# babbu3682/MTD-GAN

Hardware: NVIDIA B200
Metric: train patches/s (64x64, bs20/GPU) (higher is better)
Workload: dtype f32

## Files before the change

include/mtdgan_b200.h:

```cpp
#ifndef MTDGAN_B200_H_
#define MTDGAN_B200_H_

#ifdef __cplusplus
extern "C" {
#endif

#define MTD_ACT_NONE_C 0
#define MTD_ACT_RELU_C 1
#define MTD_ACT_LEAKY_C 2

int mtd_abi_version(void);
int mtd_device_ok(void);
long long mtd_kernel_launch_count(void);
int mtd_set_pdl(int enabled);

int mtd_conv_pack_fwd(const float* w_ref, int transposed, int Cout, int Cin, int kh, int kw, float* out, void* stream);
int mtd_conv_pack_dgrad(const float* w_ref, int transposed, int Cout, int Cin, int kh, int kw, int stride, float* out,
                        void* stream);
int mtd_conv_pack_fwd_blocked(const float* w_ref, int transposed, int Cout, int Cin, int kh, int kw, int tf32, float* out,
                              void* stream);
int mtd_conv_pack_dgrad_blocked(const float* w_ref, int transposed, int Cout, int Cin, int kh, int kw, int stride, int tf32,
                                float* out, void* stream);
int mtd_conv_pack_batch_begin(void);
int mtd_conv_pack_batch_end(void* stream);
int mtd_conv_fwd(const float* x1, const float* x2, const float* wp, const float* bias, const float* scale, int scale_group,
                 float* y,
                 float* aux, const float* add1, const float* add2, int B, int H, int W, int C1, int C2, int N, int kh,
                 int kw, int stride, int pad, int pre_act, int post_act, float slope, void* stream);
int mtd_conv_dgrad(const float* dz, const float* wpd, float* dx, const float* scale, int scale_group, const float* add1,
                   const float* add2, const float* mask_src, int mask_act, float slope, int B, int H, int W, int Cin,
                   int Cout, int kh, int kw, int stride, int pad, void* stream);
int mtd_conv_wgrad(const float* x1, const float* x2, const float* dz, float* gp, int B, int H, int W, int C1, int C2,
                   int N, int kh, int kw, int stride, int pad, void* stream);
int mtd_conv_wgrad_finish(const float* gp, float* dw_ref, int transposed, int Cout, int Cin, int kh, int kw,
                          const float* w_ref, const float* u, const float* v, const float* inv_sigma, void* scratch,
                          void* stream);
int mtd_act_bwd_sn(const float* dy, const float* y, float* dz, float* dbias, const float* bias, double* zw,
                   const float* dz_scale, int groups, long long M, int N, int act, float slope, void* stream);
int mtd_wgrad_finish_chunk_elems(int taps, int cin);
int mtd_wgrad_finish_batched(const void* seg_tab, int n_segs, const void* dot_chunks, int n_dot_chunks, const void* head_chunks,
                             int n_head_chunks, double* dots, void* stream);
int mtd_act_bwd(const float* dy, const float* y, float* dz, float* dbias, int dbias_zeroed, long long M, int N, int act, float slope,
                void* stream);

int mtd_conv_fwd_tc_supported(int B, int H, int W, int C1, int C2, int N, int kh, int kw, int stride, int pad);
int mtd_tc_set_version(int version);
int mtd_tc_set_tuning(int bn, int sk_per);
int mtd_tc_set_c32(int enabled);
int mtd_tc_set_halo(int enabled);
int mtd_round_tf32(float* p, long long n, void* stream);
int mtd_conv_fwd_tc(const float* x1, const float* x2, const float* wp, const float* bias, const float* scale, int scale_group,
                    float* y,
                    float* aux, const float* add1, const float* add2, int B, int H, int W, int C1, int C2, int N, int kh,
                    int kw, int stride, int pad, int pre_act, int post_act, float slope, int passes, float* ws, long long ws_floats,
                    void* stream);
int mtd_conv_dgrad_tc(const float* dz, const float* wpd, float* dx, const float* scale, int scale_group, const float* add1,
                      const float* add2,
                      const float* mask_src, int mask_act, float slope, int B, int H, int W, int Cin, int Cout, int kh, int kw,
                      int stride, int pad, int passes, int cin_total, float* dx2, int c_split, float* ws, long long ws_floats,
                      void* stream);
int mtd_conv_wgrad_tc_supported(int B, int H, int W, int C1, int C2, int N, int kh, int kw, int stride, int pad);
int mtd_conv_wgrad_tc(const float* x1, const float* x2, const float* dz, float* gp, int B, int H, int W, int C1, int C2, int N,
                      int kh, int kw, int stride, int pad, int passes, void* stream);
int mtd_split_tf32(float* hi, float* lo, long long n, void* stream);

int mtd_fft_supported(int H, int W, int C);
long long mtd_fft_spec_elems(int B, int H, int W, int C);
long long mtd_fft_bwd_part_elems(int B, int W);
int mtd_fft_rows_fwd(const float* x, float* spec, int B, int H, int W, int C, void* stream);
int mtd_fft_cols_mix(const float* spec_in, float* spec_out, const float* w, const float* bias, int B, int H, int W,
                     int C, void* stream);
int mtd_fft_rows_inv(const float* spec, const float* add1, const float* add2, float* out, int B, int H, int W, int C,
                     void* stream);
int mtd_fft_cols_mix_bwd(const float* spec_x, const float* spec_g, float* spec_out, const float* w, const float* bias,
                         float* part, float* dw, float* db, int B, int H, int W, int C, void* stream);

int mtd_sn_rows_per_wtu_item(void);
int mtd_sn_power_iter(const void* layer_tab, int n_layers, const void* work_wtu, int n_wtu, const void* work_wv,
                      int n_wv, float* t_ws, long long t_elems, float* s_ws, float* u_snap, float* v_snap,
                      float* inv_sigma, int update, float eps, void* stream);

int mtd_upsample2x_fwd(const float* in, float* out, int B, int H, int W, int C, void* stream);
int mtd_upsample2x_bwd(const float* dout, float* din, int B, int H, int W, int C, void* stream);
int mtd_pixel_shuffle2(const float* in, float* out, int B, int H, int W, int C, int backward, void* stream);
int mtd_layout_transpose(const float* in, float* out, int B, int C, int HW, int to_nhwc, void* stream);
int mtd_clip01_fwd(const float* x, float* y, long long n, void* stream);
int mtd_clip01_bwd(const float* x, const float* dy, float* dx, long long n, void* stream);
int mtd_mul(const float* a, const float* b, float* out, long long n, void* stream);
int mtd_add3(const float* a, const float* b, const float* c, float* out, long long n, void* stream);

int mtd_nds_mask(const float* x, const float* y, unsigned char* mask, long long n, void* stream);
// ... 32 lines not shown
```

mtd-gan_b200/csrc/conv_simt.cu:

```cuda
#include <algorithm>
#include <string.h>
#include <vector>
#include "common.cuh"
#include "mtdgan_b200.h"

namespace {

constexpr int kMaxTaps = 16;

struct ConvArgs {
  const float* src1;
  const float* src2;
  int C1, C2;
  int B, H, W;
  const float* wp;
  int N, T;
  int Ho, Wo;
  int sy, sx;
  int dy[kMaxTaps], dx[kMaxTaps];
  float* out;
  int outH, outW, omy, omx, ooy, oox;
  const float* scale;
  long long scale_span;
  const float* bias;
// ... 1018 lines not shown
#pragma unroll
        for (int j = 0; j < TC; ++j) acc[i][j] = fmaf(av[i], bv[j], acc[i][j]);
    }
    if (has_next) store_tiles(buf ^ 1);
    __syncthreads();
    buf ^= 1;
  }
#pragma unroll
  for (int i = 0; i < TN; ++i) {
    int n = n0 + ty * TN + i;
    if (n >= a.N) continue;
#pragma unroll
    for (int j = 0; j < TC; ++j) {
      int c = c0 + tx * TC + j;
      if (c >= Ctot) continue;
      float* dst = a.gp + ((size_t)n * a.T + t) * Ctot + c;
      if (a.splits > 1) atomicAdd(dst, acc[i][j]);
      else *dst = acc[i][j];
    }
  }
}

int launch_wgrad(WgradArgs& a, cudaStream_t st) {
  const int Ctot = a.C1 + a.C2;
  const int M = a.B * a.Ho * a.Wo;
  if (M <= 0 || a.N <= 0 || Ctot <= 0 || a.T <= 0 || a.T > kMaxTaps) return MTD_EINVAL;
  bool vec = (a.C1 % 4 == 0) && (a.C2 % 4 == 0) && (a.N % 4 == 0) && mtd_aligned16(a.src1) &&
             mtd_aligned16(a.dz) && (a.C2 == 0 || mtd_aligned16(a.src2));
  bool thin_n = a.N <= 16, thin_c = Ctot <= 16;
  int BN = thin_n ? 16 : 64, BC = thin_c ? 16 : 64;
  dim3 grid((a.N + BN - 1) / BN, (Ctot + BC - 1) / BC, a.T);
  int tiles = grid.x * grid.y * grid.z;
  int target = 4 * mtd_sm_count();
  int splits = 1;
  if (tiles < target) splits = std::min((target + tiles - 1) / tiles, std::max(1, M / 64));
  if (splits > 256) splits = 256;
  a.splits = splits;
  grid.z = a.T * splits;
  if (splits > 1) MTD_CUDA(cudaMemsetAsync(a.gp, 0, (size_t)a.N * a.T * Ctot * sizeof(float), st));
#define WG_LAUNCH(TN_, TC_)                                                              \
  do {                                                                                   \
    if (vec) mtd_launch(conv_wgrad_kernel<TN_, TC_, true>, grid, 256, 0, st, a);                 \
    else mtd_launch(conv_wgrad_kernel<TN_, TC_, false>, grid, 256, 0, st, a);                    \
  } while (0)
  if (thin_n && thin_c) WG_LAUNCH(1, 1);
  else if (thin_n) WG_LAUNCH(1, 4);
  else if (thin_c) WG_LAUNCH(4, 1);
  else WG_LAUNCH(4, 4);
#undef WG_LAUNCH
  MTD_CHECK_LAUNCH();
  return MTD_OK;
}

__global__ void act_bwd_kernel(const float* __restrict__ dy, const float* __restrict__ y, float* __restrict__ dz,
                               float* __restrict__ dbias, size_t total, int N, int act, float slope) {
  mtd_pdl_prologue();
  extern __shared__ float colsum[];
  if (dbias) {
    for (int i = threadIdx.x; i < N; i += blockDim.x) colsum[i] = 0.f;
    __syncthreads();
  }
  size_t i = (size_t)blockIdx.x * blockDim.x + threadIdx.x;
  size_t stride = (size_t)gridDim.x * blockDim.x;
  const bool fixed = dbias && (stride % (size_t)N == 0);
  float priv = 0.f;
  for (; i < total; i += stride) {
    float g = dy[i];
    if (act != MTD_ACT_NONE) g *= mtd_act_grad(__ldg(y + i), act, slope);
    if (dz) dz[i] = g;
    if (dbias) {
      if (fixed) priv += g;
      else atomicAdd(&colsum[i % N], g);
    }
  }
  if (dbias) {
    if (fixed) {
      size_t first = (size_t)blockIdx.x * blockDim.x + threadIdx.x;
      atomicAdd(&colsum[first % N], priv);
    }
    __syncthreads();
    for (int c = threadIdx.x; c < N; c += blockDim.x) {
      float v = colsum[c];
      if (v != 0.f) atomicAdd(dbias + c, v);
    }
  }
}

__global__ void __launch_bounds__(256) act_bwd_v4_kernel(const float4* __restrict__ dy, const float4* __restrict__ y,
                                                         float4* __restrict__ dz, float* __restrict__ dbias, size_t total4,
                                                         int N4, int act, float slope) {
  mtd_pdl_prologue();
  extern __shared__ float colsum[];
  if (dbias) {
    for (int i = threadIdx.x; i < 4 * N4; i += blockDim.x) colsum[i] = 0.f;
    __syncthreads();
  }
  size_t i = (size_t)blockIdx.x * blockDim.x + threadIdx.x;
  const size_t stride = (size_t)gridDim.x * blockDim.x;
  const bool fixed = dbias && (stride % (size_t)N4 == 0);
  float4 priv = make_float4(0.f, 0.f, 0.f, 0.f);
  const size_t first = i;
  for (; i < total4; i += stride) {
    float4 g = __ldcs(dy + i);
    if (act != MTD_ACT_NONE) {
      const float4 t = __ldcs(y + i);
      g.x *= mtd_act_grad(t.x, act, slope); g.y *= mtd_act_grad(t.y, act, slope);
      g.z *= mtd_act_grad(t.z, act, slope); g.w *= mtd_act_grad(t.w, act, slope);
    }
    if (dz) dz[i] = g;
    if (dbias) {
      if (fixed) { priv.x += g.x; priv.y += g.y; priv.z += g.z; priv.w += g.w; }
      else {
        float* cs = colsum + 4 * (i % N4);
        atomicAdd(cs, g.x); atomicAdd(cs + 1, g.y); atomicAdd(cs + 2, g.z); atomicAdd(cs + 3, g.w);
      }
    }
  }
  if (dbias) {
    if (fixed && first < total4) {
      float* cs = colsum + 4 * (first % N4);
      atomicAdd(cs, priv.x); atomicAdd(cs + 1, priv.y); atomicAdd(cs + 2, priv.z); atomicAdd(cs + 3, priv.w);
    }
    __syncthreads();
    for (int c = threadIdx.x; c < 4 * N4; c += blockDim.x) {
      float v = colsum[c];
      if (v != 0.f) atomicAdd(dbias + c, v);
    }
  }
}

__global__ void __launch_bounds__(256) act_bwd_sn_kernel(const float4* __restrict__ dy, const float4* __restrict__ y,
                                                         float4* __restrict__ dz, float* __restrict__ dbias,
                                                         const float4* __restrict__ bias, double* __restrict__ zw,
                                                         const float* __restrict__ dz_scale, size_t total4, size_t group4,
                                                         int N4, int act, float slope) {
  mtd_pdl_prologue();
  extern __shared__ float colsum[];
  __shared__ double red[32];
  if (dbias) {
    for (int i = threadIdx.x; i < 4 * N4; i += blockDim.x) colsum[i] = 0.f;
    __syncthreads();
  }
  size_t i = (size_t)blockIdx.x * blockDim.x + threadIdx.x;
  const size_t stride = (size_t)gridDim.x * blockDim.x;
  const size_t first = i;
  const float4 b4 = (bias && first < total4) ? __ldg(bias + first % N4) : make_float4(0.f, 0.f, 0.f, 0.f);
  const float inv_slope = 1.f / slope;
  float4 priv = make_float4(0.f, 0.f, 0.f, 0.f);
  double part[4] = {0.0, 0.0, 0.0, 0.0};
  for (; i < total4; i += stride) {
    float4 g = __ldcs(dy + i);
    const float4 t = __ldcs(y + i);
    float4 yp = t;
    if (act == MTD_ACT_LEAKY) {
      g.x *= t.x > 0.f ? 1.f : slope; g.y *= t.y > 0.f ? 1.f : slope; g.z *= t.z > 0.f ? 1.f : slope; g.w *= t.w > 0.f ? 1.f : slope;
      yp.x = t.x > 0.f ? t.x : t.x * inv_slope; yp.y = t.y > 0.f ? t.y : t.y * inv_slope;
      yp.z = t.z > 0.f ? t.z : t.z * inv_slope; yp.w = t.w > 0.f ? t.w : t.w * inv_slope;
    }
    const int gi = (i >= group4) + (i >= 2 * group4) + (i >= 3 * group4);
    if (dz) {
      const float a = dz_scale ? __ldg(dz_scale + gi) : 1.f;
      dz[i] = make_float4(g.x * a, g.y * a, g.z * a, g.w * a);
    }
    priv.x += g.x; priv.y += g.y; priv.z += g.z; priv.w += g.w;
    const float d = g.x * (yp.x - b4.x) + g.y * (yp.y - b4.y) + g.z * (yp.z - b4.z) + g.w * (yp.w - b4.w);
    part[gi] += (double)d;
  }
  if (dbias) {
    if (first < total4) {
      float* cs = colsum + 4 * (first % N4);
      atomicAdd(cs, priv.x); atomicAdd(cs + 1, priv.y); atomicAdd(cs + 2, priv.z); atomicAdd(cs + 3, priv.w);
    }
    __syncthreads();
    for (int c = threadIdx.x; c < 4 * N4; c += blockDim.x) {
      float v = colsum[c];
      if (v != 0.f) atomicAdd(dbias + c, v);
    }
  }
  const int ngroups = (int)((total4 + group4 - 1) / group4);
  for (int k = 0; k < ngroups && k < 4; ++k) {
    const double r = block_sum(part[k], red);
    if (threadIdx.x == 0 && r != 0.0) atomicAdd(zw + k, r);
  }
}

void tap_table_fwd(int* dy, int* dx, int kh, int kw, int pad) {
  for (int ky = 0; ky < kh; ++ky)
    for (int kx = 0; kx < kw; ++kx) {
      dy[ky * kw + kx] = ky - pad;
      dx[ky * kw + kx] = kx - pad;
    }
}

}

extern "C" {

static int g_pack_blocked = 0;
static int g_pack_tf32 = 0;

int mtd_conv_pack_fwd(const float* w_ref, int transposed, int Cout, int Cin, int kh, int kw, float* out, void* stream) {
  MTD_REQUIRE(w_ref && out && Cout > 0 && Cin > 0 && kh > 0 && kw > 0 && kh * kw <= kMaxTaps);
  PackArgs p;
  fwd_mapping(p, transposed, Cout, Cin, kh, kw);
  p.blocked = g_pack_blocked; p.tf32 = g_pack_tf32; p.lo_off = (long long)Cout * Cin * kh * kw;
  if (p.blocked) MTD_REQUIRE(Cout % 32 == 0 && Cin % 32 == 0);
  return pack_launch(w_ref, out, p, (cudaStream_t)stream);
}

int mtd_conv_pack_dgrad(const float* w_ref, int transposed, int Cout, int Cin, int kh, int kw, int stride, float* out,
                        void* stream) {
  MTD_REQUIRE(w_ref && out && Cout > 0 && Cin > 0 && kh * kw <= kMaxTaps);
  PackArgs f;
  fwd_mapping(f, transposed, Cout, Cin, kh, kw);
  cudaStream_t st = (cudaStream_t)stream;
  if (stride == 1) {
    PackArgs p;
    p.N = Cin; p.T = kh * kw; p.C = Cout; p.sN = f.sC; p.sC = f.sN;
    for (int t = 0; t < p.T; ++t) p.toff[t] = f.toff[t];
    p.blocked = g_pack_blocked; p.tf32 = g_pack_tf32; p.lo_off = (long long)Cout * Cin * kh * kw;
    if (p.blocked) MTD_REQUIRE(Cout % 32 == 0 && Cin % 32 == 0);
    return pack_launch(w_ref, out, p, st);
  }
  MTD_REQUIRE(stride == 2 && kh == 4 && kw == 4 && !transposed);
  for (int py = 0; py < 2; ++py)
    for (int px = 0; px < 2; ++px) {
      PackArgs p;
      p.blocked = g_pack_blocked; p.tf32 = g_pack_tf32; p.lo_off = (long long)Cout * Cin * kh * kw;
      if (p.blocked) MTD_REQUIRE(Cout % 32 == 0 && Cin % 32 == 0);
      p.N = Cin; p.T = 4; p.C = Cout; p.sN = f.sC; p.sC = f.sN;
      for (int a = 0; a < 2; ++a)
// ... 137 lines not shown
  if (stride == 1 && a.Ho == H && a.Wo == W && (N == 1 || Ctot == 1) && (N == 1 ? Ctot : N) <= 256) {
    cudaStream_t st = (cudaStream_t)stream;
    ThinWgArgs w{};
    w.B = B; w.H = H; w.W = W; w.T = a.T; w.out = gp;
    if (N == 1 && Ctot > 1) {
      w.V1 = x1; w.V2 = x2; w.J1 = C1; w.J2 = C2; w.s = dz;
      for (int t = 0; t < a.T; ++t) { w.dy[t] = -a.dy[t]; w.dx[t] = -a.dx[t]; }
      w.st_t = Ctot; w.st_j = 1;
    } else {
      w.V1 = dz; w.V2 = nullptr; w.J1 = N; w.J2 = 0; w.s = x1;
      for (int t = 0; t < a.T; ++t) { w.dy[t] = a.dy[t]; w.dx[t] = a.dx[t]; }
      w.st_t = Ctot; w.st_j = (long long)a.T * Ctot;
    }
    const long long M = (long long)B * H * W;
    int blocks = mtd_sm_count() * 4;
    if (blocks > M / 64 + 1) blocks = (int)(M / 64 + 1);
    w.pix_per_block = (int)((M + blocks - 1) / blocks);
    blocks = (int)((M + w.pix_per_block - 1) / w.pix_per_block);
    MTD_CUDA(cudaMemsetAsync(gp, 0, (size_t)N * a.T * Ctot * sizeof(float), st));
    const int J = w.J1 + w.J2;
    const bool vec4 = (w.J1 % 4 == 0) && (w.J2 % 4 == 0) && J >= 4 && mtd_aligned16(w.V1) && (!w.V2 || mtd_aligned16(w.V2));
    const size_t smem = (size_t)a.T * J * sizeof(float);
    if (vec4) mtd_launch(thin_wgrad_kernel<true>, blocks, 256, smem, st, w);
    else mtd_launch(thin_wgrad_kernel<false>, blocks, 256, smem, st, w);
    MTD_CHECK_LAUNCH();
    return MTD_OK;
  }
  return launch_wgrad(a, (cudaStream_t)stream);
}

int mtd_conv_wgrad_finish(const float* gp, float* dw_ref, int transposed, int Cout, int Cin, int kh, int kw,
                          const float* w_ref, const float* u, const float* v, const float* inv_sigma, void* scratch,
                          void* stream) {
  MTD_REQUIRE(gp && dw_ref && Cout > 0 && Cin > 0 && kh * kw <= kMaxTaps);
  cudaStream_t st = (cudaStream_t)stream;
  UnpackArgs a{};
  fwd_mapping(a.p, transposed, Cout, Cin, kh, kw);
  size_t total = (size_t)Cout * Cin * kh * kw;
  int blocks = (int)std::min<size_t>((total + 255) / 256, (size_t)mtd_sm_count() * 16);
  if (inv_sigma) {
    MTD_REQUIRE(w_ref && u && v && scratch && !transposed);
    double* acc = (double*)scratch;
    MTD_CUDA(cudaMemsetAsync(acc, 0, 8, st));
    mtd_launch(dot_packed_ref_kernel, blocks, 256, 0, st, gp, w_ref, acc, a.p);
    MTD_CHECK_LAUNCH();
    a.inv_sigma = inv_sigma; a.dotgw = acc; a.u = u; a.v = v;
    a.sn_rows = Cout; a.sn_cols = (long long)Cin * kh * kw;
  }
  mtd_launch(unpack_grad_kernel, blocks, 256, 0, st, gp, dw_ref, a);
  MTD_CHECK_LAUNCH();
  return MTD_OK;
}

int mtd_act_bwd(const float* dy, const float* y, float* dz, float* dbias, int dbias_zeroed, long long M, int N, int act,
                float slope, void* stream) {
  MTD_REQUIRE(dy && M > 0 && N > 0 && (act == MTD_ACT_NONE || y));
  cudaStream_t st = (cudaStream_t)stream;
  size_t total = (size_t)M * N;
  if (N % 4 == 0 && mtd_aligned16(dy) && (!y || mtd_aligned16(y)) && (!dz || mtd_aligned16(dz))) {
    const size_t total4 = total / 4;
    const int N4 = N / 4;
    int blocks = (int)std::min<size_t>((total4 + 255) / 256, (size_t)mtd_sm_count() * 4);
    if (dbias) {
      MTD_REQUIRE(N <= 8192);
      if (!dbias_zeroed) MTD_CUDA(cudaMemsetAsync(dbias, 0, (size_t)N * sizeof(float), st));
      size_t stride = (size_t)blocks * 256;
      if (stride % N4 != 0 && (size_t)N4 <= stride) {
        size_t s2 = stride / N4 * N4;
        if (s2 % 256 == 0 && s2 > 0) blocks = (int)(s2 / 256);
      } else if ((size_t)N4 > stride) {
        blocks = (N4 + 255) / 256;
      }
    }
    mtd_launch(act_bwd_v4_kernel, blocks, 256, dbias ? N * sizeof(float) : 0, st, reinterpret_cast<const float4*>(dy),
               reinterpret_cast<const float4*>(y), reinterpret_cast<float4*>(dz), dbias, total4, N4, act, slope);
    MTD_CHECK_LAUNCH();
    return MTD_OK;
  }
  int blocks = (int)std::min<size_t>((total + 255) / 256, (size_t)mtd_sm_count() * 8);
  if (dbias) {
    MTD_REQUIRE(N <= 8192);
    if (!dbias_zeroed) MTD_CUDA(cudaMemsetAsync(dbias, 0, (size_t)N * sizeof(float), st));
    size_t stride = (size_t)blocks * 256;
    if (stride % N != 0 && (size_t)N <= stride) {
      size_t s2 = stride / N * N;
      if (s2 % 256 == 0 && s2 > 0) blocks = (int)(s2 / 256);
    } else if ((size_t)N > stride) {
      blocks = (N + 255) / 256;
    }
  }
  mtd_launch(act_bwd_kernel, blocks, 256, dbias ? N * sizeof(float) : 0, st, dy, y, dz, dbias, total, N, act, slope);
  MTD_CHECK_LAUNCH();
  return MTD_OK;
}

int mtd_act_bwd_sn(const float* dy, const float* y, float* dz, float* dbias, const float* bias, double* zw,
                   const float* dz_scale, int groups, long long M, int N, int act, float slope, void* stream) {
  MTD_REQUIRE(dy && y && zw && M > 0 && N > 0 && N % 4 == 0 && N <= 8192 && groups >= 1 && groups <= 4 && M % groups == 0);
  MTD_REQUIRE(act == MTD_ACT_NONE || act == MTD_ACT_LEAKY);
  MTD_REQUIRE(mtd_aligned16(dy) && mtd_aligned16(y) && (!dz || mtd_aligned16(dz)) && (!bias || mtd_aligned16(bias)));
  cudaStream_t st = (cudaStream_t)stream;
  const size_t total4 = (size_t)M * N / 4;
  const int N4 = N / 4;
  int blocks = (int)std::min<size_t>((total4 + 255) / 256, (size_t)mtd_sm_count() * 4);
  size_t stride = (size_t)blocks * 256;
  if ((size_t)N4 > stride) blocks = (N4 + 255) / 256;
  else if (stride % N4 != 0) {
    size_t s2 = stride / N4 * N4;
    while (s2 > 0 && s2 % 256 != 0) s2 -= N4;
    MTD_REQUIRE(s2 > 0);
    blocks = (int)(s2 / 256);
  }
  MTD_REQUIRE(((size_t)blocks * 256) % N4 == 0);
  mtd_launch(act_bwd_sn_kernel, blocks, 256, dbias ? N * sizeof(float) : 0, st, reinterpret_cast<const float4*>(dy),
             reinterpret_cast<const float4*>(y), reinterpret_cast<float4*>(dz), dbias, reinterpret_cast<const float4*>(bias), zw,
             dz_scale, total4, total4 / groups, N4, act, slope);
  MTD_CHECK_LAUNCH();
  return MTD_OK;
}

int mtd_wgrad_finish_chunk_elems(int taps, int cin) { return (int)fin_chunk_elems(taps, cin); }

int mtd_wgrad_finish_batched(const void* seg_tab, int n_segs, const void* dot_chunks, int n_dot_chunks, const void* head_chunks,
                             int n_head_chunks, double* dots, void* stream) {
  MTD_REQUIRE(seg_tab && head_chunks && dots && n_segs > 0 && n_head_chunks > 0);
  cudaStream_t st = (cudaStream_t)stream;
  if (n_dot_chunks > 0) {
    MTD_REQUIRE(dot_chunks);
    MTD_CUDA(cudaMemsetAsync(dots, 0, (size_t)n_segs * sizeof(double), st));
    mtd_launch(finish_dot_kernel, n_dot_chunks, 256, 0, st, reinterpret_cast<const FinSeg*>(seg_tab),
                                                    reinterpret_cast<const int2*>(dot_chunks), dots);
    MTD_CHECK_LAUNCH();
  }
  mtd_launch(finish_unpack_kernel, n_head_chunks, 256, 0, st, reinterpret_cast<const FinSeg*>(seg_tab),
                                                      reinterpret_cast<const int2*>(head_chunks), dots);
  MTD_CHECK_LAUNCH();
  return MTD_OK;
}

}
```

mtd-gan_b200/ops.py:

```python
from __future__ import annotations

import os
import weakref
from dataclasses import dataclass


import torch
from torch.autograd import Function

from . import _ext
from ._ext import call, fptr, ptr, stream

ACT_NONE, ACT_RELU, ACT_LEAKY = 0, 1, 2
LEAK = 0.2


def _empty(shape, like):
    return torch.empty(shape, dtype=torch.float32, device=like.device)


_pack_cache: dict = {}


def clear_pack_cache():
# ... 165 lines not shown
        _zw_slab = [torch.zeros(8192, dtype=torch.float64, device=like.device), 0]
    t, off = _zw_slab
    if off + n > t.numel():
        return None
    _zw_slab[1] = off + n
    return t[off:off + n]


def _dbias_alloc(n: int, like):
    global _bias_slab
    if _finish_queue is not None:
        if _bias_slab is None:
            _bias_slab = [torch.zeros(_BIAS_SLAB_FLOATS, dtype=torch.float32, device=like.device), 0]
        t, off = _bias_slab
        step = (n + 63) // 64 * 64
        if off + step <= t.numel():
            _bias_slab[1] = off + step
            return t[off:off + n], 1
    return _empty((n,), like), 0


def _flush_finish(groups):
    first = next(iter(groups.values()))
    dev = first[0].device
    rows, dot_numels, head_numels, heads, rowdims = [], [], [], [], []
    for dw, insts in groups.values():
        base = len(rows)
        heads.append(base)
        head_numels.append(dw.numel())
        for k, (gp, w, u, v, inv, cfg, zwp, flags) in enumerate(insts):
            T = cfg.kh * cfg.kw
            sN, sC, flip = (T, cfg.cout * T, 1) if cfg.transposed else (cfg.cin * T, T, 0)
            sn = inv is not None
            rows.append([gp.data_ptr() if gp is not None else 0, dw.data_ptr(), w.data_ptr() if sn else 0,
                         u.data_ptr() if sn else 0, v.data_ptr() if sn else 0, inv.data_ptr() if sn else 0, cfg.cout, T, cfg.cin,
                         sN, sC, flip | flags,
                         cfg.cin * T, base + k, base + k + 1 if k + 1 < len(insts) else -1, zwp])
            dot_numels.append(gp.numel() if (sn and not zwp and gp is not None) else 0)
            rowdims.append((T, cfg.cin))
    key = (tuple(dot_numels), tuple(heads), tuple(rowdims), str(dev))
    ent = _fin_chunk_cache.get(key)
    if ent is None:
        ck = [_ext.load().mtd_wgrad_finish_chunk_elems(t, c) for t, c in rowdims]
        dchunks = [[s_, off] for s_, n in enumerate(dot_numels) for off in range(0, n, ck[s_])]
        hchunks = [[h, off] for h, n in zip(heads, head_numels) for off in range(0, n, ck[h])]
        ent = (_ext.device_table(dchunks, torch.int32, dev) if dchunks else None, len(dchunks),
               _ext.device_table(hchunks, torch.int32, dev), len(hchunks))
        _fin_chunk_cache[key] = ent
    seg = _ext.device_table(rows, torch.int64, dev)
    dots = torch.empty(len(rows), dtype=torch.float64, device=dev)
    call("mtd_wgrad_finish_batched", ptr(seg), len(rows), ptr(ent[0]), ent[1], ptr(ent[2]), ent[3], ptr(dots), stream())


@dataclass(frozen=True)
class ConvCfg:
    cin: int
    cout: int
    kh: int = 3
    kw: int = 3
    stride: int = 1
    pad: int = 1
    transposed: int = 0
    pre_act: int = ACT_NONE
    post_act: int = ACT_NONE
    slope: float = LEAK
    fuse_add1_is_input: bool = False
    freeze: bool = False


_USE_TC = os.environ.get("MTDGAN_CONV", "auto")
tc_launches = 0


_TC_PASSES = 1 if os.environ.get("MTDGAN_TF32", "x3") == "x1" else 3
_WGRAD_PASSES = 3 if os.environ.get("MTDGAN_WGRAD_TF32", "x1") == "x3" else 1


_TC_VERSION = 1


def set_tc_version(version: int) -> int:
    global _TC_VERSION
    prev = _ext.load().mtd_tc_set_version(int(version))
    _TC_VERSION = int(version)
    return prev


def _tc_version() -> int:
    return _TC_VERSION


def set_wgrad_passes(passes: int):
    global _WGRAD_PASSES
    assert passes in (1, 3)
    _WGRAD_PASSES = passes


def set_conv_mode(mode: str, passes: int | None = None):
    global _USE_TC, _TC_PASSES
    assert mode in ("auto", "simt")
    _USE_TC = mode
    if passes is not None:
        assert passes in (1, 3)
        _TC_PASSES = passes


# ... 84 lines not shown


def _conv_dgrad_launch_cat(dz, weight, dx1, dx2, scale, B, H, W, C1, C2, cfg: ConvCfg) -> bool:
    if (cfg.stride != 1 or C1 % 32 or C2 % 32 or _tc_version() != 1
            or not _tc_ok(B, H, W, cfg.cout, 0, C1 + C2, cfg.kh, cfg.kw, 1, cfg.pad)):
        return False
    global tc_launches
    tc_launches += 1
    wpd = _packed(weight, _tc_kind("dgrad"), cfg)
    ws = _tc_workspace(dx1.device)
    call("mtd_conv_dgrad_tc", fptr(dz), fptr(wpd), fptr(dx1), fptr(scale), _scale_group(scale, B), None, None, None, 0, cfg.slope,
         B, H, W, C1 + C2, cfg.cout, cfg.kh, cfg.kw, 1, cfg.pad, _TC_PASSES, cfg.cin, fptr(dx2), C1, fptr(ws), ws.numel(), stream())
    return True


class ConvFn(Function):

    @staticmethod
    def forward(ctx, x1, x2, weight, bias, inv_sigma, u, v, add1, add2, cfg: ConvCfg):
        B, H, W, C1 = x1.shape
        C2 = 0 if x2 is None else x2.shape[3]
        assert C1 + C2 == cfg.cin, (C1, C2, cfg)
        Ho = (H + 2 * cfg.pad - cfg.kh) // cfg.stride + 1
        Wo = (W + 2 * cfg.pad - cfg.kw) // cfg.stride + 1
        y = _empty((B, Ho, Wo, cfg.cout), x1)
        has_add = add1 is not None or add2 is not None
        need_graph = any(ctx.needs_input_grad)
        aux = _empty(y.shape, x1) if (need_graph and cfg.pre_act != ACT_NONE and has_add) else None
        _conv_forward_launch(x1, x2, weight, bias, inv_sigma, y, aux, add1, add2, cfg)
        ctx.cfg = cfg
        ctx.has_add = has_add
        ctx.weight_obj = weight
        ctx.shapes = (B, H, W, C1, C2)
        ctx.save_for_backward(x1, x2, weight, inv_sigma, u, v, y, aux, bias)
        return y

    @staticmethod
    def backward(ctx, dy):
        cfg: ConvCfg = ctx.cfg
        x1, x2, weight, inv_sigma, u, v, y, aux, bias = ctx.saved_tensors
        weight = ctx.weight_obj
        B, H, W, C1, C2 = ctx.shapes
        need = list(ctx.needs_input_grad)
        if cfg.freeze:
            need[2] = need[3] = False
        dy = dy.contiguous()
        M = dy.numel() // cfg.cout
        st = stream()
        g1 = dy
        if cfg.post_act != ACT_NONE:
            g1 = _empty(dy.shape, dy)
            call("mtd_act_bwd", fptr(dy), fptr(y), fptr(g1), None, 0, M, cfg.cout, cfg.post_act, cfg.slope, st)
        d_add = g1 if ctx.has_add else None
        dbias, dbz = _dbias_alloc(cfg.cout, dy) if need[3] else (None, 0)
        want_w = need[2] and _wgrad_wanted(weight)
        G = 1 if inv_sigma is None else inv_sigma.numel()
        zw = None
        deferred = _finish_queue is not None and not torch.is_anomaly_enabled()
        if (want_w and inv_sigma is not None and deferred and cfg.post_act == ACT_NONE and not ctx.has_add
                and cfg.pre_act in (ACT_NONE, ACT_LEAKY) and cfg.cout % 4 == 0 and G <= 4):
            zw = _zw_alloc(G, dy)
        if zw is not None:
            if dbias is not None and not dbz:
                dbias.zero_()
            dz = _empty(dy.shape, dy)
            call("mtd_act_bwd_sn", fptr(g1), fptr(y), fptr(dz), fptr(dbias), fptr(bias), zw.data_ptr(), fptr(inv_sigma), G, M,
                 cfg.cout, cfg.pre_act, cfg.slope, st)
        elif cfg.pre_act != ACT_NONE:
            pre_out = aux if aux is not None else y
            dz = _empty(dy.shape, dy)
            call("mtd_act_bwd", fptr(g1), fptr(pre_out), fptr(dz), fptr(dbias), dbz, M, cfg.cout, cfg.pre_act, cfg.slope, st)
        else:
            dz = g1
            if dbias is not None:
                call("mtd_act_bwd", fptr(g1), None, None, fptr(dbias), dbz, M, cfg.cout, ACT_NONE, cfg.slope, st)
        dw = None
        if want_w:
            Bg = B // G
            insts = []
            if zw is not None:
                gp = _empty((weight.numel(),), dy)
                if _WGRAD_SIDE:
                    _on_side_stream(lambda: _conv_wgrad_launch(x1, x2, dz, gp, B, H, W, C1, C2, cfg), x1, x2, dz, gp)
                else:
                    _conv_wgrad_launch(x1, x2, dz, gp, B, H, W, C1, C2, cfg)
                for g in range(G):
                    insts.append((gp if g == 0 else None, weight.detach(), u[g] if u.dim() == 2 else u, v[g] if v.dim() == 2 else v,
                                  inv_sigma[g:g + 1], cfg, zw.data_ptr() + 8 * g, 2 if g == 0 else 4))
            else:
                for g in range(G):
                    gp = _empty((weight.numel(),), dy)
                    if G == 1:
                        if _WGRAD_SIDE and deferred:
                            _on_side_stream(lambda gp=gp: _conv_wgrad_launch(x1, x2, dz, gp, B, H, W, C1, C2, cfg), x1, x2, dz, gp)
                        else:
                            _conv_wgrad_launch(x1, x2, dz, gp, B, H, W, C1, C2, cfg)
                        insts.append((gp, weight.detach(), None if u is None else u.reshape(-1),
                                      None if v is None else v.reshape(-1), inv_sigma, cfg, 0, 0))
                    else:
                        sl = slice(g * Bg, (g + 1) * Bg)
                        _conv_wgrad_launch(x1[sl], None if x2 is None else x2[sl], dz[sl], gp, Bg, H, W, C1, C2, cfg)
                        insts.append((gp, weight.detach(), u[g], v[g], inv_sigma[g:g + 1], cfg, 0, 0))
            if deferred:
                grp = _finish_queue.get(weight.data_ptr())
                if grp is None:
                    dw = torch.empty_like(weight)
                    _finish_queue[weight.data_ptr()] = (dw, insts)
                else:
                    grp[1].extend(insts)
            else:
                for k, (gp, wd, ug, vg, inv_g, _, _zw, _fl) in enumerate(insts):
                    part = torch.empty_like(weight)
                    scratch = torch.empty(4, dtype=torch.float32, device=dy.device) if inv_g is not None else None
                    call("mtd_conv_wgrad_finish", fptr(gp), fptr(part), cfg.transposed, cfg.cout, cfg.cin, cfg.kh, cfg.kw,
                         fptr(wd) if inv_g is not None else None, fptr(ug), fptr(vg), fptr(inv_g), ptr(scratch), st)
# ... 216 lines not shown
```

mtd-gan_b200/weight_methods.py:

```python
from __future__ import annotations

import random
from typing import Dict, List, Optional, Sequence, Tuple

import torch

from . import _ext
from . import distributed as mdist
from ._ext import call, fptr, ptr, stream
from .ops import deferred_wgrad_finish, wgrad_only_for


def draw_visit_orders(n_tasks: int, rng=None) -> List[List[int]]:
    shuffle = (rng or random).shuffle
    idx = list(range(n_tasks))
    orders = []
    for _ in range(n_tasks):
        shuffle(idx)
        orders.append(list(idx))
    return orders


_chunk_cache: Dict[Tuple[int, ...], Tuple[torch.Tensor, int]] = {}


def _chunk_table(numels: Sequence[int], device) -> Tuple[torch.Tensor, int]:
    key = (tuple(numels), str(device))
    ent = _chunk_cache.get(key)
    if ent is None:
        ck = _ext.load().mtd_pcgrad_chunk_elems()
        rows = [[s, off] for s, n in enumerate(numels) for off in range(0, n, ck)]
        ent = (_ext.device_table(rows, torch.int32, device), len(rows))
        _chunk_cache[key] = ent
    return ent


def _float_bits(x: float) -> int:
    return int(torch.tensor(x, dtype=torch.float32).view(torch.int32).item())


def pcgrad_merge(task_grads: Sequence[Sequence[Optional[torch.Tensor]]], orders, mean: bool,
                 seg_scales: Optional[Sequence[float]] = None, return_debug: bool = False):
    T = len(task_grads)
    P = len(task_grads[0])
    ref = next(g for tg in task_grads for g in tg if g is not None)
    device = ref.device
    shapes, numels = [], []
    for p in range(P):
        g = next((task_grads[k][p] for k in range(T) if task_grads[k][p] is not None), None)
        if g is None:
            raise _ext.MtdError("pcgrad_merge: parameter without any gradient needs an explicit shape")
        shapes.append(g.shape)
        numels.append(g.numel())
    flat = torch.empty(sum(numels), dtype=torch.float32, device=device)
    rows, off = [], 0
    keep = []
    for p in range(P):
        row = []
        for k in range(4):
            g = task_grads[k][p] if k < T else None
            if g is not None:
                g = g.contiguous()
                keep.append(g)
# ... 40 lines not shown
    chunks, n_chunks = _chunk_table([out.numel()], dev)
    ords = orders if isinstance(orders, torch.Tensor) else _ext.device_table(orders, torch.int32, dev)
    coef = torch.empty(4, dtype=torch.float32, device=dev)
    call("mtd_pcgrad_solve_combine", ptr(seg), ptr(chunks), n_chunks, T, ptr(ords), 1 if mean else 0, ptr(gram), fptr(coef),
         None, None, stream())
    return out


class WeightMethod:
    def __init__(self, n_tasks: int, device: torch.device):
        super().__init__()
        self.n_tasks = n_tasks
        self.device = device

    def get_weighted_loss(self, losses, **kwargs):
        raise NotImplementedError

    def backward(self, losses, shared_parameters=None, task_specific_parameters=None, last_shared_parameters=None,
                 representation=None, **kwargs):
        loss, extra_outputs = self.get_weighted_loss(
            losses=losses, shared_parameters=shared_parameters, task_specific_parameters=task_specific_parameters,
            last_shared_parameters=last_shared_parameters, representation=representation, **kwargs)
        loss.backward()
        return loss, extra_outputs

    def __call__(self, losses, **kwargs):
        return self.backward(losses, **kwargs)

    def parameters(self) -> List[torch.Tensor]:
        return []


class PCGrad(WeightMethod):

    def __init__(self, n_tasks: int, device: torch.device, reduction="sum"):
        super().__init__(n_tasks, device=device)
        assert reduction in ["mean", "sum"]
        self.reduction = reduction

    def get_weighted_loss(self, losses, shared_parameters=None, task_specific_parameters=None, **kwargs):
        raise NotImplementedError

    def _set_pc_grads(self, losses, shared_parameters, task_specific_parameters=None):
        if isinstance(shared_parameters, torch.Tensor):
            shared_parameters = [shared_parameters]
        shared_parameters = list(shared_parameters)
        if task_specific_parameters is not None:
            if isinstance(task_specific_parameters, torch.Tensor):
                task_specific_parameters = [task_specific_parameters]
            task_specific_parameters = list(task_specific_parameters)
        if mdist.active():
            return self._set_pc_grads_distributed(losses, shared_parameters, task_specific_parameters)
        shared_grads = []
        with wgrad_only_for(shared_parameters):
            for l in losses:
                with deferred_wgrad_finish():
                    shared_grads.append(torch.autograd.grad(l, shared_parameters, retain_graph=True))
        merged = self._project_conflicting(shared_grads)
        for p, g in zip(shared_parameters, merged):
            p.grad = g
        if task_specific_parameters is not None:
            with wgrad_only_for(task_specific_parameters), deferred_wgrad_finish():
                ts_grads = torch.autograd.grad(losses.sum(), task_specific_parameters)
            for p, g in zip(task_specific_parameters, ts_grads):
                p.grad = g

    def _set_pc_grads_distributed(self, losses, shared_parameters, task_specific_parameters):
        ts_pending = None
        if task_specific_parameters is not None:
            with wgrad_only_for(task_specific_parameters), deferred_wgrad_finish():
                ts_grads = torch.autograd.grad(losses.sum(), task_specific_parameters, retain_graph=True)
            ts_pending = mdist.allreduce_mean_list_async(ts_grads)
        pipe = mdist.ShardedPCGrad()
        n = len(losses)
        with wgrad_only_for(shared_parameters):
            for k, l in enumerate(losses):
                with deferred_wgrad_finish():
                    g = torch.autograd.grad(l, shared_parameters, retain_graph=(k + 1 < n))
                pipe.submit(g)
        orders = self.refresh_orders(shared_parameters[0].device)
        merged = pipe.finish(orders, self.reduction == "mean", _cuda_gram, _cuda_solve_combine)
        for p, g in zip(shared_parameters, merged):
            p.grad = g
        if ts_pending is not None:
            for p, g in zip(task_specific_parameters, ts_pending.wait()):
                p.grad = g

    def refresh_orders(self, device):
        T = self.n_tasks
        if getattr(self, "_orders_host", None) is None or self._orders_dev.device != torch.device(device):
            self._orders_host = torch.zeros(T * T, dtype=torch.int32).pin_memory()
            self._orders_dev = torch.zeros(T * T, dtype=torch.int32, device=device)
        self.draw_orders_host()
        self._orders_dev.copy_(self._orders_host, non_blocking=True)
        return self._orders_dev

    def draw_orders_host(self):
        orders = draw_visit_orders(self.n_tasks)
        self._orders_host.copy_(torch.tensor(orders, dtype=torch.int32).reshape(-1))
        return orders

    def _project_conflicting(self, grads: List[Tuple[torch.Tensor]]):
        assert len(grads) == self.n_tasks
        orders = self.refresh_orders(grads[0][0].device)
        if mdist.active():
            return mdist.pcgrad_sharded(grads, orders, self.reduction == "mean", _cuda_gram, _cuda_solve_combine)
        return pcgrad_merge(grads, orders, mean=(self.reduction == "mean"))

    def backward(self, losses, parameters=None, shared_parameters=None, task_specific_parameters=None, **kwargs):
        self._set_pc_grads(losses, shared_parameters, task_specific_parameters)
        return None, {}


class WeightMethods:

    def __init__(self, method: str, n_tasks: int, device: torch.device, **kwargs):
        assert method in list(METHODS.keys()), f"unknown method {method}."
        self.method = METHODS[method](n_tasks=n_tasks, device=device, **kwargs)

    def get_weighted_loss(self, losses, **kwargs):
        return self.method.get_weighted_loss(losses, **kwargs)

    def backward(self, losses, **kwargs):
        return self.method.backward(losses, **kwargs)

    def __ceil__(self, losses, **kwargs):
        return self.backward(losses, **kwargs)

    def parameters(self):
        return self.method.parameters()


# ... 2 lines not shown
```

Before: 584.9.

## Fold task-specific parameter gradients into per-task shared backward passes

Removes the separate backward pass over the summed loss for task-specific parameters in PCGrad. Each per-task backward now accumulates the pre-activation gradients of the task-specific convolutions into a buffer through a new fused act-backward kernel that also sums bias and spectral-norm terms. Weight gradients are issued once, on the last pass, from the accumulated buffer. The cost is extra accumulation traffic and buffers, plus a more complex control flow tied to autograd node identity and the pass order.

```diff
diff --git a/include/mtdgan_b200.h b/include/mtdgan_b200.h
--- a/include/mtdgan_b200.h
+++ b/include/mtdgan_b200.h
@@ -37,6 +37,8 @@
                           void* stream);
 int mtd_act_bwd_sn(const float* dy, const float* y, float* dz, float* dbias, const float* bias, double* zw,
                    const float* dz_scale, int groups, long long M, int N, int act, float slope, void* stream);
+int mtd_act_bwd_acc(const float* dy, const float* y, float* dz, float* acc, int acc_first, float* dbias, const float* bias,
+                    double* zw, const float* inv_sigma, int groups, long long M, int N, int act, float slope, void* stream);
 int mtd_wgrad_finish_chunk_elems(int taps, int cin);
 int mtd_wgrad_finish_batched(const void* seg_tab, int n_segs, const void* dot_chunks, int n_dot_chunks, const void* head_chunks,
                              int n_head_chunks, double* dots, void* stream);
diff --git a/mtd-gan_b200/csrc/conv_simt.cu b/mtd-gan_b200/csrc/conv_simt.cu
--- a/mtd-gan_b200/csrc/conv_simt.cu
+++ b/mtd-gan_b200/csrc/conv_simt.cu
@@ -1094,8 +1094,18 @@
   return MTD_OK;
 }
 
+struct ActFold {
+  float* acc;
+  const float* scale;
+  const float* bias;
+  double* zw;
+  size_t group;
+  int first;
+};
+
+template <bool FOLD>
 __global__ void act_bwd_kernel(const float* __restrict__ dy, const float* __restrict__ y, float* __restrict__ dz,
-                               float* __restrict__ dbias, size_t total, int N, int act, float slope) {
+                               float* __restrict__ dbias, size_t total, int N, int act, float slope, ActFold f) {
   mtd_pdl_prologue();
   extern __shared__ float colsum[];
   if (dbias) {
@@ -1106,9 +1116,22 @@
   size_t stride = (size_t)gridDim.x * blockDim.x;
   const bool fixed = dbias && (stride % (size_t)N == 0);
   float priv = 0.f;
+  double part[4] = {0.0, 0.0, 0.0, 0.0};
   for (; i < total; i += stride) {
     float g = dy[i];
-    if (act != MTD_ACT_NONE) g *= mtd_act_grad(__ldg(y + i), act, slope);
+    if constexpr (FOLD) {
+      const float t = (act != MTD_ACT_NONE || f.zw) ? __ldg(y + i) : 0.f;
+      if (act != MTD_ACT_NONE) g *= mtd_act_grad(t, act, slope);
+      const int gi = (i >= f.group) + (i >= 2 * f.group) + (i >= 3 * f.group);
+      const float a = f.scale ? __ldg(f.scale + gi) : 1.f;
+      f.acc[i] = f.first ? g * a : f.acc[i] + g * a;
+      if (f.zw) {
+        const float yp = (act == MTD_ACT_LEAKY && !(t > 0.f)) ? t * (1.f / slope) : t;
+        part[gi] += (double)(g * (yp - (f.bias ? __ldg(f.bias + i % N) : 0.f)));
+      }
+    } else {
+      if (act != MTD_ACT_NONE) g *= mtd_act_grad(__ldg(y + i), act, slope);
+    }
     if (dz) dz[i] = g;
     if (dbias) {
       if (fixed) priv += g;
@@ -1124,6 +1147,16 @@
     for (int c = threadIdx.x; c < N; c += blockDim.x) {
       float v = colsum[c];
       if (v != 0.f) atomicAdd(dbias + c, v);
+    }
+  }
+  if constexpr (FOLD) {
+    if (f.zw) {
+      __shared__ double red[32];
+      const int ngroups = (int)((total + f.group - 1) / f.group);
+      for (int k = 0; k < ngroups && k < 4; ++k) {
+        const double r = block_sum(part[k], red);
+        if (threadIdx.x == 0 && r != 0.0) atomicAdd(f.zw + k, r);
+      }
     }
   }
 }
@@ -1171,11 +1204,13 @@
   }
 }
 
+template <bool FOLD>
 __global__ void __launch_bounds__(256) act_bwd_sn_kernel(const float4* __restrict__ dy, const float4* __restrict__ y,
                                                          float4* __restrict__ dz, float* __restrict__ dbias,
                                                          const float4* __restrict__ bias, double* __restrict__ zw,
                                                          const float* __restrict__ dz_scale, size_t total4, size_t group4,
-                                                         int N4, int act, float slope) {
+                                                         int N4, int act, float slope, float4* __restrict__ acc,
+                                                         int acc_first) {
   mtd_pdl_prologue();
   extern __shared__ float colsum[];
   __shared__ double red[32];
@@ -1192,7 +1227,7 @@
   double part[4] = {0.0, 0.0, 0.0, 0.0};
   for (; i < total4; i += stride) {
     float4 g = __ldcs(dy + i);
-    const float4 t = __ldcs(y + i);
+    const float4 t = (FOLD && !y) ? make_float4(0.f, 0.f, 0.f, 0.f) : __ldcs(y + i);
     float4 yp = t;
     if (act == MTD_ACT_LEAKY) {
       g.x *= t.x > 0.f ? 1.f : slope; g.y *= t.y > 0.f ? 1.f : slope; g.z *= t.z > 0.f ? 1.f : slope; g.w *= t.w > 0.f ? 1.f : slope;
@@ -1200,13 +1235,25 @@
       yp.z = t.z > 0.f ? t.z : t.z * inv_slope; yp.w = t.w > 0.f ? t.w : t.w * inv_slope;
     }
     const int gi = (i >= group4) + (i >= 2 * group4) + (i >= 3 * group4);
-    if (dz) {
+    if constexpr (FOLD) {
+      if (dz) dz[i] = g;
+      const float a = dz_scale ? __ldg(dz_scale + gi) : 1.f;
+      const float4 s = make_float4(g.x * a, g.y * a, g.z * a, g.w * a);
+      if (acc_first) {
+        acc[i] = s;
+      } else {
+        const float4 o = acc[i];
+        acc[i] = make_float4(o.x + s.x, o.y + s.y, o.z + s.z, o.w + s.w);
+      }
+    } else if (dz) {
       const float a = dz_scale ? __ldg(dz_scale + gi) : 1.f;
       dz[i] = make_float4(g.x * a, g.y * a, g.z * a, g.w * a);
     }
     priv.x += g.x; priv.y += g.y; priv.z += g.z; priv.w += g.w;
-    const float d = g.x * (yp.x - b4.x) + g.y * (yp.y - b4.y) + g.z * (yp.z - b4.z) + g.w * (yp.w - b4.w);
-    part[gi] += (double)d;
+    if (!FOLD || zw) {
+      const float d = g.x * (yp.x - b4.x) + g.y * (yp.y - b4.y) + g.z * (yp.z - b4.z) + g.w * (yp.w - b4.w);
+      part[gi] += (double)d;
+    }
   }
   if (dbias) {
     if (first < total4) {
@@ -1219,6 +1266,7 @@
       if (v != 0.f) atomicAdd(dbias + c, v);
     }
   }
+  if (FOLD && !zw) return;
   const int ngroups = (int)((total4 + group4 - 1) / group4);
   for (int k = 0; k < ngroups && k < 4; ++k) {
     const double r = block_sum(part[k], red);
@@ -1462,6 +1510,32 @@
   return MTD_OK;
 }
 
+static int act_bwd_scalar_blocks(size_t total, int N, bool colsums) {
+  int blocks = (int)std::min<size_t>((total + 255) / 256, (size_t)mtd_sm_count() * 8);
+  if (colsums) {
+    size_t stride = (size_t)blocks * 256;
+    if (stride % N != 0 && (size_t)N <= stride) {
+      size_t s2 = stride / N * N;
+      if (s2 % 256 == 0 && s2 > 0) blocks = (int)(s2 / 256);
+    } else if ((size_t)N > stride) {
+      blocks = (N + 255) / 256;
+    }
+  }
+  return blocks;
+}
+
+static int act_bwd_sn_blocks(size_t total4, int N4) {
+  int blocks = (int)std::min<size_t>((total4 + 255) / 256, (size_t)mtd_sm_count() * 4);
+  size_t stride = (size_t)blocks * 256;
+  if ((size_t)N4 > stride) blocks = (N4 + 255) / 256;
+  else if (stride % N4 != 0) {
+    size_t s2 = stride / N4 * N4;
+    while (s2 > 0 && s2 % 256 != 0) s2 -= N4;
+    blocks = (int)(s2 / 256);
+  }
+  return ((size_t)blocks * 256) % N4 == 0 ? blocks : 0;
+}
+
 int mtd_act_bwd(const float* dy, const float* y, float* dz, float* dbias, int dbias_zeroed, long long M, int N, int act,
                 float slope, void* stream) {
   MTD_REQUIRE(dy && M > 0 && N > 0 && (act == MTD_ACT_NONE || y));
@@ -1487,19 +1561,12 @@
     MTD_CHECK_LAUNCH();
     return MTD_OK;
   }
-  int blocks = (int)std::min<size_t>((total + 255) / 256, (size_t)mtd_sm_count() * 8);
   if (dbias) {
     MTD_REQUIRE(N <= 8192);
     if (!dbias_zeroed) MTD_CUDA(cudaMemsetAsync(dbias, 0, (size_t)N * sizeof(float), st));
-    size_t stride = (size_t)blocks * 256;
-    if (stride % N != 0 && (size_t)N <= stride) {
-      size_t s2 = stride / N * N;
-      if (s2 % 256 == 0 && s2 > 0) blocks = (int)(s2 / 256);
-    } else if ((size_t)N > stride) {
-      blocks = (N + 255) / 256;
-    }
-  }
-  mtd_launch(act_bwd_kernel, blocks, 256, dbias ? N * sizeof(float) : 0, st, dy, y, dz, dbias, total, N, act, slope);
+  }
+  mtd_launch(act_bwd_kernel<false>, act_bwd_scalar_blocks(total, N, dbias != nullptr), 256, dbias ? N * sizeof(float) : 0, st,
+             dy, y, dz, dbias, total, N, act, slope, ActFold{});
   MTD_CHECK_LAUNCH();
   return MTD_OK;
 }
@@ -1512,19 +1579,36 @@
   cudaStream_t st = (cudaStream_t)stream;
   const size_t total4 = (size_t)M * N / 4;
   const int N4 = N / 4;
-  int blocks = (int)std::min<size_t>((total4 + 255) / 256, (size_t)mtd_sm_count() * 4);
-  size_t stride = (size_t)blocks * 256;
-  if ((size_t)N4 > stride) blocks = (N4 + 255) / 256;
-  else if (stride % N4 != 0) {
-    size_t s2 = stride / N4 * N4;
-    while (s2 > 0 && s2 % 256 != 0) s2 -= N4;
-    MTD_REQUIRE(s2 > 0);
-    blocks = (int)(s2 / 256);
-  }
-  MTD_REQUIRE(((size_t)blocks * 256) % N4 == 0);
-  mtd_launch(act_bwd_sn_kernel, blocks, 256, dbias ? N * sizeof(float) : 0, st, reinterpret_cast<const float4*>(dy),
+  const int blocks = act_bwd_sn_blocks(total4, N4);
+  MTD_REQUIRE(blocks > 0);
+  mtd_launch(act_bwd_sn_kernel<false>, blocks, 256, dbias ? N * sizeof(float) : 0, st, reinterpret_cast<const float4*>(dy),
              reinterpret_cast<const float4*>(y), reinterpret_cast<float4*>(dz), dbias, reinterpret_cast<const float4*>(bias), zw,
-             dz_scale, total4, total4 / groups, N4, act, slope);
+             dz_scale, total4, total4 / groups, N4, act, slope, static_cast<float4*>(nullptr), 0);
+  MTD_CHECK_LAUNCH();
+  return MTD_OK;
+}
+
+int mtd_act_bwd_acc(const float* dy, const float* y, float* dz, float* acc, int acc_first, float* dbias, const float* bias,
+                    double* zw, const float* inv_sigma, int groups, long long M, int N, int act, float slope, void* stream) {
+  MTD_REQUIRE(dy && acc && M > 0 && N > 0 && N <= 8192 && groups >= 1 && groups <= 4 && M % groups == 0);
+  MTD_REQUIRE(y || (act == MTD_ACT_NONE && !zw));
+  MTD_REQUIRE(!zw || act == MTD_ACT_NONE || act == MTD_ACT_LEAKY);
+  cudaStream_t st = (cudaStream_t)stream;
+  const size_t total = (size_t)M * N;
+  if (N % 4 == 0 && mtd_aligned16(dy) && mtd_aligned16(acc) && (!y || mtd_aligned16(y)) && (!dz || mtd_aligned16(dz)) &&
+      (!bias || mtd_aligned16(bias))) {
+    const size_t total4 = total / 4;
+    const int N4 = N / 4;
+    const int blocks = act_bwd_sn_blocks(total4, N4);
+    MTD_REQUIRE(blocks > 0);
+    mtd_launch(act_bwd_sn_kernel<true>, blocks, 256, dbias ? N * sizeof(float) : 0, st, reinterpret_cast<const float4*>(dy),
+               reinterpret_cast<const float4*>(y), reinterpret_cast<float4*>(dz), dbias, reinterpret_cast<const float4*>(bias),
+               zw, inv_sigma, total4, total4 / groups, N4, act, slope, reinterpret_cast<float4*>(acc), acc_first);
+  } else {
+    const ActFold f{acc, inv_sigma, bias, zw, total / groups, acc_first};
+    mtd_launch(act_bwd_kernel<true>, act_bwd_scalar_blocks(total, N, dbias != nullptr), 256, dbias ? N * sizeof(float) : 0,
+               st, dy, y, dz, dbias, total, N, act, slope, f);
+  }
   MTD_CHECK_LAUNCH();
   return MTD_OK;
 }
diff --git a/mtd-gan_b200/ops.py b/mtd-gan_b200/ops.py
--- a/mtd-gan_b200/ops.py
+++ b/mtd-gan_b200/ops.py
@@ -241,6 +241,129 @@
     call("mtd_wgrad_finish_batched", ptr(seg), len(rows), ptr(ent[0]), ent[1], ptr(ent[2]), ent[3], ptr(dots), stream())
 
 
+_fold = None
+
+
+class _FoldRec:
+
+    def __init__(self, node, weight, x1, x2, dz_like, bias_grad, inv_sigma, u, v, zw, cfg, shapes):
+        self.node = node
+        self.weight, self.x1, self.x2 = weight, x1, x2
+        self.acc = _empty(dz_like.shape, dz_like)
+        self.bias_grad, self.inv_sigma, self.u, self.v, self.zw = bias_grad, inv_sigma, u, v, zw
+        self.cfg, self.shapes = cfg, shapes
+        self.gp = None
+
+
+class fold_task_grads:
+
+    def __init__(self, params):
+        self.params = list(params)
+        self.ptrs = {p.data_ptr() for p in self.params}
+        self.records = {}
+        self.bias_grads = {}
+        self.last_pass = False
+        self.grads = None
+        self._fslab = self._dslab = None
+
+    def __enter__(self):
+        global _fold
+        self.prev, _fold = _fold, self
+        return self
+
+    def __exit__(self, *exc):
+        global _fold
+        _fold = self.prev
+        if exc[0] is None:
+            self.grads = self._finish()
+        self.records = {}
+        return False
+
+    def wants(self, weight) -> bool:
+        return weight.data_ptr() in self.ptrs
+
+    def _zeros(self, n, dtype, like):
+        f = dtype == torch.float32
+        slab = self._fslab if f else self._dslab
+        if slab is None:
+            slab = [torch.zeros(1 << 16 if f else 1024, dtype=dtype, device=like.device), 0]
+            if f:
+                self._fslab = slab
+            else:
+                self._dslab = slab
+        step = (n + 63) // 64 * 64
+        if slab[1] + step > slab[0].numel():
+            return torch.zeros(n, dtype=dtype, device=like.device)
+        t = slab[0][slab[1]:slab[1] + n]
+        slab[1] += step
+        return t
+
+    def act_bwd(self, node, g1, pre_out, weight, bias, want_bias, inv_sigma, u, v, x1, x2, cfg: "ConvCfg", shapes, has_add):
+        sn = inv_sigma is not None
+        G = inv_sigma.numel() if sn else 1
+        rec = self.records.get(id(node))
+        first = rec is None
+        if first:
+            if sn and (has_add or cfg.post_act != ACT_NONE or cfg.pre_act not in (ACT_NONE, ACT_LEAKY) or G > 4):
+                raise _ext.MtdError(f"task-gradient fold: no kernel for a spectrally-normalised layer with {cfg}")
+            bias_grad = None
+            if want_bias:
+                bias_grad = self.bias_grads.get(bias.data_ptr())
+                if bias_grad is None:
+                    bias_grad = self.bias_grads[bias.data_ptr()] = self._zeros(cfg.cout, torch.float32, g1)
+            zw = self._zeros(G, torch.float64, g1) if sn else None
+            rec = self.records[id(node)] = _FoldRec(node, weight, x1, x2, g1, bias_grad, inv_sigma, u, v, zw, cfg, shapes)
+        act = cfg.pre_act
+        dz = _empty(g1.shape, g1) if act != ACT_NONE else g1
+        y_in = pre_out if (act != ACT_NONE or sn) else None
+        call("mtd_act_bwd_acc", fptr(g1), fptr(y_in), fptr(dz) if act != ACT_NONE else None, fptr(rec.acc), 1 if first else 0,
+             fptr(rec.bias_grad), fptr(bias) if sn else None, ptr(rec.zw), fptr(inv_sigma), G, g1.numel() // cfg.cout,
+             cfg.cout, act, cfg.slope, stream())
+        if self.last_pass:
+            self._issue_wgrad(rec)
+        return dz
+
+    def _issue_wgrad(self, rec):
+        if rec.gp is not None:
+            return
+        B, H, W, C1, C2 = rec.shapes
+        rec.gp = gp = _empty((rec.weight.numel(),), rec.acc)
+        launch = lambda: _conv_wgrad_launch(rec.x1, rec.x2, rec.acc, gp, B, H, W, C1, C2, rec.cfg)
+        if _WGRAD_SIDE and _finish_queue is not None and not torch.is_anomaly_enabled():
+            _on_side_stream(launch, rec.x1, rec.x2, rec.acc, gp)
+        else:
+            launch()
+
+    def _finish(self):
+        groups = {}
+        for rec in self.records.values():
+            self._issue_wgrad(rec)
+            w = rec.weight.detach()
+            if rec.inv_sigma is not None:
+                u, v, G = rec.u, rec.v, rec.inv_sigma.numel()
+                insts = [(rec.gp if g == 0 else None, w, u[g] if u.dim() == 2 else u, v[g] if v.dim() == 2 else v,
+                          rec.inv_sigma[g:g + 1], rec.cfg, rec.zw.data_ptr() + 8 * g, 2 if g == 0 else 4) for g in range(G)]
+            else:
+                insts = [(rec.gp, w, None, None, None, rec.cfg, 0, 0)]
+            grp = groups.get(w.data_ptr())
+            if grp is None:
+                groups[w.data_ptr()] = (torch.empty_like(w), insts)
+            else:
+                grp[1].extend(insts)
+        _join_side_stream()
+        if groups:
+            _flush_finish(groups)
+        out = []
+        for p in self.params:
+            g = groups.get(p.data_ptr())
+            g = g[0] if g is not None else self.bias_grads.get(p.data_ptr())
+            if g is None:
+                raise _ext.MtdError(f"task-gradient fold: parameter of shape {tuple(p.shape)} was reached by no backward "
+                                    "pass (it is not used in the graph of the losses)")
+            out.append(g)
+        return out
+
+
 @dataclass(frozen=True)
 class ConvCfg:
     cin: int
@@ -431,6 +554,11 @@
             g1 = _empty(dy.shape, dy)
             call("mtd_act_bwd", fptr(dy), fptr(y), fptr(g1), None, 0, M, cfg.cout, cfg.post_act, cfg.slope, st)
         d_add = g1 if ctx.has_add else None
+        folded = _fold is not None and need[2] and _fold.wants(weight)
+        if folded:
+            dz = _fold.act_bwd(ctx, g1, aux if aux is not None else y, weight, bias, need[3], inv_sigma, u, v, x1, x2, cfg,
+                               ctx.shapes, ctx.has_add)
+            need[2] = need[3] = False
         dbias, dbz = _dbias_alloc(cfg.cout, dy) if need[3] else (None, 0)
         want_w = need[2] and _wgrad_wanted(weight)
         G = 1 if inv_sigma is None else inv_sigma.numel()
@@ -439,7 +567,9 @@
         if (want_w and inv_sigma is not None and deferred and cfg.post_act == ACT_NONE and not ctx.has_add
                 and cfg.pre_act in (ACT_NONE, ACT_LEAKY) and cfg.cout % 4 == 0 and G <= 4):
             zw = _zw_alloc(G, dy)
-        if zw is not None:
+        if folded:
+            pass
+        elif zw is not None:
             if dbias is not None and not dbz:
                 dbias.zero_()
             dz = _empty(dy.shape, dy)
diff --git a/mtd-gan_b200/weight_methods.py b/mtd-gan_b200/weight_methods.py
--- a/mtd-gan_b200/weight_methods.py
+++ b/mtd-gan_b200/weight_methods.py
@@ -8,7 +8,7 @@
 from . import _ext
 from . import distributed as mdist
 from ._ext import call, fptr, ptr, stream
-from .ops import deferred_wgrad_finish, wgrad_only_for
+from .ops import deferred_wgrad_finish, fold_task_grads, wgrad_only_for
 
 
 def draw_visit_orders(n_tasks: int, rng=None) -> List[List[int]]:
@@ -155,32 +155,27 @@
         if mdist.active():
             return self._set_pc_grads_distributed(losses, shared_parameters, task_specific_parameters)
         shared_grads = []
-        with wgrad_only_for(shared_parameters):
-            for l in losses:
+        with wgrad_only_for(shared_parameters), fold_task_grads(task_specific_parameters or []) as fold:
+            for k, l in enumerate(losses):
+                fold.last_pass = k + 1 == len(losses)
                 with deferred_wgrad_finish():
-                    shared_grads.append(torch.autograd.grad(l, shared_parameters, retain_graph=True))
+                    shared_grads.append(torch.autograd.grad(l, shared_parameters, retain_graph=not fold.last_pass))
         merged = self._project_conflicting(shared_grads)
         for p, g in zip(shared_parameters, merged):
             p.grad = g
         if task_specific_parameters is not None:
-            with wgrad_only_for(task_specific_parameters), deferred_wgrad_finish():
-                ts_grads = torch.autograd.grad(losses.sum(), task_specific_parameters)
-            for p, g in zip(task_specific_parameters, ts_grads):
+            for p, g in zip(task_specific_parameters, fold.grads):
                 p.grad = g
 
     def _set_pc_grads_distributed(self, losses, shared_parameters, task_specific_parameters):
-        ts_pending = None
-        if task_specific_parameters is not None:
-            with wgrad_only_for(task_specific_parameters), deferred_wgrad_finish():
-                ts_grads = torch.autograd.grad(losses.sum(), task_specific_parameters, retain_graph=True)
-            ts_pending = mdist.allreduce_mean_list_async(ts_grads)
         pipe = mdist.ShardedPCGrad()
-        n = len(losses)
-        with wgrad_only_for(shared_parameters):
+        with wgrad_only_for(shared_parameters), fold_task_grads(task_specific_parameters or []) as fold:
             for k, l in enumerate(losses):
+                fold.last_pass = k + 1 == len(losses)
                 with deferred_wgrad_finish():
-                    g = torch.autograd.grad(l, shared_parameters, retain_graph=(k + 1 < n))
+                    g = torch.autograd.grad(l, shared_parameters, retain_graph=not fold.last_pass)
                 pipe.submit(g)
+        ts_pending = mdist.allreduce_mean_list_async(fold.grads) if task_specific_parameters is not None else None
         orders = self.refresh_orders(shared_parameters[0].device)
         merged = pipe.finish(orders, self.reduction == "mean", _cuda_gram, _cuda_solve_combine)
         for p, g in zip(shared_parameters, merged):
```

After: 634.0, median of 6. +8.4%, better.
